# SewoongLab/PLeaS-Merging

Measured on NVIDIA B200. Metric: rn50_pair_merge_calib_samples_per_s, higher is better.
Workload: dtype f32

## Files before the change

### include/pleas_b200.h

```cpp
#ifndef PLEAS_B200_H
#define PLEAS_B200_H

#include <stdint.h>

#ifdef __cplusplus
extern "C" {
#endif

#define PLB_OK 0
#define PLB_EINVAL (-1)
#define PLB_ESIZE (-2)
#define PLB_EALIGN (-3)

#define PLB_MODE_INNER 0
#define PLB_MODE_NEG_CDIST 1
#define PLB_MODE_CORR 2

int plb_version(void);
const char *plb_last_error_string(void);


int64_t plb_plane_bytes(int64_t rows, int64_t K, int32_t *row_groups, int32_t *k_blocks);

int plb_pack_split(const float *x, int64_t outer, int64_t src_rows, int64_t inner,
                   const int64_t *row_index, int64_t rows,
                   float *hi, float *lo, int32_t row_groups, int32_t kb_offset,
                   double *row_sumsq, double *row_sum, void *stream);

int plb_pack_split_pair(const float *xa, const float *xb, int64_t outer, int64_t src_rows, int64_t inner,
                        float *hi_a, float *lo_a, float *hi_b, float *lo_b, int32_t row_groups,
                        int32_t kb_offset, double *sumsq_a, double *sumsq_b, void *stream);
int plb_pack_split_pair_sums(const float *xa, const float *xb, int64_t outer, int64_t src_rows, int64_t inner,
                             float *hi_a, float *lo_a, float *hi_b, float *lo_b, int32_t row_groups,
                             int32_t kb_offset, double *sumsq_a, double *sumsq_b, double *sum_a,
                             double *sum_b, void *stream);

int plb_pack_im2col(const float *x1, const float *x2, int64_t N, int64_t cin_src, int64_t H, int64_t W,
                    const int32_t *chan1, const int32_t *chan2, const float *scale1, const float *scale2,
                    int64_t cmerged, int32_t kh, int32_t kw, int32_t stride_h, int32_t stride_w,
                    int32_t pad_h, int32_t pad_w, int32_t dil_h, int32_t dil_w, int64_t Ho, int64_t Wo,
                    int32_t ones_row, float *hi, float *lo, int32_t row_groups, int32_t kb_offset,
                    void *stream);

int plb_gram_direct(const float *x, const float *y, int64_t outer, int64_t C, int64_t inner,
                    float *partial, int32_t splits, int32_t chain_kb, double *row_sumsq_x,
                    double *row_sumsq_y, void *stream);

int plb_gram_tma(const float *x, const float *y, int64_t outer, int64_t C, int64_t inner,
                 float *partial, int32_t splits, int32_t chain_kb, double *row_sumsq_x,
                 double *row_sumsq_y, double *row_sum_x, double *row_sum_y, void *stream);

int plb_debug_set_trace(unsigned long long *dev_buf);

int plb_gram_tma_geometry(int64_t C, int32_t *cta_group, int32_t *m_tiles, int32_t *n_tiles,
                          int32_t *ld_m, int32_t *ld_n);

typedef struct PlbGemmProblem {
  const float *a_hi, *a_lo;
  const float *b_hi, *b_lo;
  float *partial;
  int32_t a_row_groups, b_row_groups;
  int32_t k_blocks;
  int32_t m_tiles, n_tiles, splits;
  int32_t cta_begin;
  int32_t symmetric;
} PlbGemmProblem;

int plb_gemm_grouped(const PlbGemmProblem *problems_dev, int32_t n_problems, int32_t total_ctas,
                     int32_t bn, int32_t impl, void *stream);

int plb_cross_finalize(const float *partial, int32_t splits, int64_t ld_m, int64_t ld_n,
                       int64_t M, int64_t N, const double *qa, const double *qb, int32_t mode,
                       float *cost, double *cost64, int64_t ldc, int32_t accumulate, int32_t sym_bn,
                       void *stream);

typedef struct PlbFinalizeTap {
  const float *partial;
  const double *qa, *qb;
  const double *sa, *sb;
  int64_t ld_m, ld_n, K;
  int32_t splits;
  int32_t n_affine;
  const double *affine;
} PlbFinalizeTap;
typedef struct PlbFinalizeGroup {
  float *cost;
  int64_t ldc;
  int32_t n, tap_begin, tap_end, block_begin;
} PlbFinalizeGroup;
int plb_cross_finalize_grouped(const PlbFinalizeTap *taps_dev, const PlbFinalizeGroup *groups_dev,
                               int32_t n_groups, int32_t total_blocks, int32_t mode, int32_t accumulate,
                               void *stream);

int plb_cross_finalize_corr(const float *partial, int32_t splits, int64_t ld_m, int64_t ld_n,
                            int64_t M, int64_t N, const double *qa, const double *qb,
                            const double *sa, const double *sb, int64_t K, float *cost, int64_t ldc,
                            int32_t accumulate, void *stream);

int plb_lap_solve_batched(const float *const *cost, const int32_t *n, const int32_t *ld,
                          int64_t *const *col4row, double *objective, int32_t *status,
                          int32_t n_problems, int32_t max_n, int32_t maximize, void *stream);

int plb_lap_solve_batched_warm(const float *const *cost, const int32_t *n, const int32_t *ld,
                               int64_t *const *col4row, double *objective, int32_t *status,
                               int32_t n_problems, int32_t max_n, int32_t maximize,
                               const double *const *v_in, double v_scale, double *const *v_out, void *stream);


int plb_get_blocks(const float *cost, int64_t ldc, const int64_t *perm, int32_t n, float ratio,
                   int32_t identity, int64_t *q_merged, int64_t *p_merged, int64_t *q_sep,
                   int64_t *p_sep, int32_t *counts, void *stream);

int plb_block_merge(const float *w1, const float *w2, int64_t O, int64_t I, int64_t R,
                    const int64_t *bo1, const int64_t *bo2, const int64_t *bo1c, const int64_t *bo2c,
                    int64_t no, int64_t mo,
                    const int64_t *bi1, const int64_t *bi2, const int64_t *bi1c, const int64_t *bi2c,
                    int64_t ni, int64_t mi, int32_t in_axis_only, float *out, void *stream);

int plb_gather_axis(const float *in, float *out, int64_t outer, int64_t n, int64_t inner,
                    const int64_t *P, void *stream);

int plb_compose_perm(const int64_t *a, const int64_t *b, int64_t *out, int64_t n, void *stream);

int plb_wm_progress(const float *A, int64_t ld, const int64_t *P, int32_t n, int32_t *flag,
                    double *gain, void *stream);

int plb_conv_debug_set_trace(unsigned long long *dev_buf);
int64_t plb_conv_packed_floats(int64_t Cout, int64_t Cin, int32_t KH, int32_t KW);
int plb_conv_pack_weights(const float *w, int64_t Cout, int64_t Cin, int32_t KH, int32_t KW, float *packed,
                          void *stream);

int plb_conv2d_forward(const float *const *x, const float *const *packed_w, const float *const *bias,
                       float *const *out, int32_t nprob, int64_t NB, int64_t Cin, int64_t IH, int64_t IW,
                       int64_t Cout, int32_t KH, int32_t KW, int32_t stride, int32_t pad_h, int32_t pad_w,
                       void *stream);

int plb_conv2d_affine_forward(const float *const *x, const float *const *packed_w, const float *const *bias,
                              float *const *out, const float *const *scale_shift, float *const *out2,
                              int32_t relu, int32_t nprob, int64_t NB, int64_t Cin, int64_t IH, int64_t IW,
                              int64_t Cout, int32_t KH, int32_t KW, int32_t stride, int32_t pad_h, int32_t pad_w,
                              void *stream);

int plb_chol_solve(double *G, int64_t n, double *B, int64_t nrhs, double ridge, int32_t *info,
                   void *stream);

#ifdef __cplusplus
}
#endif
#endif
```

### pleas_merging_b200/_native.py

```python
import ctypes
import os

_HERE = os.path.dirname(os.path.abspath(__file__))
LIB_PATH = os.path.join(_HERE, "lib", "libpleas_b200.so")

c_i32, c_i64, c_f32, c_f64, c_ptr = ctypes.c_int32, ctypes.c_int64, ctypes.c_float, ctypes.c_double, ctypes.c_void_p


class GemmProblem(ctypes.Structure):
    _fields_ = [
        ("a_hi", c_ptr), ("a_lo", c_ptr), ("b_hi", c_ptr), ("b_lo", c_ptr), ("partial", c_ptr),
        ("a_row_groups", c_i32), ("b_row_groups", c_i32), ("k_blocks", c_i32),
        ("m_tiles", c_i32), ("n_tiles", c_i32), ("splits", c_i32), ("cta_begin", c_i32), ("symmetric", c_i32),
    ]


class FinalizeTap(ctypes.Structure):
    _fields_ = [("partial", c_ptr), ("qa", c_ptr), ("qb", c_ptr), ("sa", c_ptr), ("sb", c_ptr),
                ("ld_m", c_i64), ("ld_n", c_i64), ("K", c_i64), ("splits", c_i32), ("n_affine", c_i32),
                ("affine", c_ptr)]


class FinalizeGroup(ctypes.Structure):
    _fields_ = [("cost", c_ptr), ("ldc", c_i64), ("n", c_i32), ("tap_begin", c_i32), ("tap_end", c_i32),
                ("block_begin", c_i32)]


_SIGNATURES = {
    "plb_version": (ctypes.c_int, []),
    "plb_last_error_string": (ctypes.c_char_p, []),
    "plb_plane_bytes": (c_i64, [c_i64, c_i64, ctypes.POINTER(c_i32), ctypes.POINTER(c_i32)]),
    "plb_pack_split": (ctypes.c_int, [c_ptr, c_i64, c_i64, c_i64, c_ptr, c_i64, c_ptr, c_ptr, c_i32, c_i32,
                                      c_ptr, c_ptr, c_ptr]),
    "plb_pack_split_pair": (ctypes.c_int, [c_ptr, c_ptr, c_i64, c_i64, c_i64, c_ptr, c_ptr, c_ptr, c_ptr, c_i32, c_i32,
                                           c_ptr, c_ptr, c_ptr]),
    "plb_gram_direct": (ctypes.c_int, [c_ptr, c_ptr, c_i64, c_i64, c_i64, c_ptr, c_i32, c_i32, c_ptr, c_ptr, c_ptr]),
    "plb_gram_tma": (ctypes.c_int, [c_ptr, c_ptr, c_i64, c_i64, c_i64, c_ptr, c_i32, c_i32, c_ptr, c_ptr, c_ptr, c_ptr,
                                    c_ptr]),
    "plb_pack_split_pair_sums": (ctypes.c_int, [c_ptr, c_ptr, c_i64, c_i64, c_i64, c_ptr, c_ptr, c_ptr, c_ptr, c_i32,
                                                c_i32, c_ptr, c_ptr, c_ptr, c_ptr, c_ptr]),
    "plb_cross_finalize_grouped": (ctypes.c_int, [c_ptr, c_ptr, c_i32, c_i32, c_i32, c_i32, c_ptr]),
    "plb_cross_finalize_corr": (ctypes.c_int, [c_ptr, c_i32, c_i64, c_i64, c_i64, c_i64, c_ptr, c_ptr, c_ptr, c_ptr,
                                               c_i64, c_ptr, c_i64, c_i32, c_ptr]),
    "plb_gram_tma_geometry": (ctypes.c_int, [c_i64, ctypes.POINTER(c_i32), ctypes.POINTER(c_i32),
                                             ctypes.POINTER(c_i32), ctypes.POINTER(c_i32), ctypes.POINTER(c_i32)]),
    "plb_debug_set_trace": (ctypes.c_int, [c_ptr]),
    "plb_pack_im2col": (ctypes.c_int, [c_ptr, c_ptr, c_i64, c_i64, c_i64, c_i64, c_ptr, c_ptr, c_ptr, c_ptr, c_i64,
                                       c_i32, c_i32, c_i32, c_i32, c_i32, c_i32, c_i32, c_i32, c_i64, c_i64, c_i32,
                                       c_ptr, c_ptr, c_i32, c_i32, c_ptr]),
    "plb_gemm_grouped": (ctypes.c_int, [c_ptr, c_i32, c_i32, c_i32, c_i32, c_ptr]),
    "plb_cross_finalize": (ctypes.c_int, [c_ptr, c_i32, c_i64, c_i64, c_i64, c_i64, c_ptr, c_ptr, c_i32, c_ptr,
                                          c_ptr, c_i64, c_i32, c_i32, c_ptr]),
    "plb_lap_solve_batched": (ctypes.c_int, [c_ptr, c_ptr, c_ptr, c_ptr, c_ptr, c_ptr, c_i32, c_i32, c_i32, c_ptr]),
    "plb_lap_solve_batched_warm": (ctypes.c_int, [c_ptr, c_ptr, c_ptr, c_ptr, c_ptr, c_ptr, c_i32, c_i32, c_i32, c_ptr,
                                                  c_f64, c_ptr, c_ptr]),
    "plb_get_blocks": (ctypes.c_int, [c_ptr, c_i64, c_ptr, c_i32, c_f32, c_i32, c_ptr, c_ptr, c_ptr, c_ptr, c_ptr,
                                      c_ptr]),
    "plb_block_merge": (ctypes.c_int, [c_ptr, c_ptr, c_i64, c_i64, c_i64, c_ptr, c_ptr, c_ptr, c_ptr, c_i64, c_i64,
                                       c_ptr, c_ptr, c_ptr, c_ptr, c_i64, c_i64, c_i32, c_ptr, c_ptr]),
    "plb_gather_axis": (ctypes.c_int, [c_ptr, c_ptr, c_i64, c_i64, c_i64, c_ptr, c_ptr]),
    "plb_compose_perm": (ctypes.c_int, [c_ptr, c_ptr, c_ptr, c_i64, c_ptr]),
    "plb_wm_progress": (ctypes.c_int, [c_ptr, c_i64, c_ptr, c_i32, c_ptr, c_ptr, c_ptr]),
    "plb_chol_solve": (ctypes.c_int, [c_ptr, c_i64, c_ptr, c_i64, c_f64, c_ptr, c_ptr]),
    "plb_conv_debug_set_trace": (ctypes.c_int, [c_ptr]),
    "plb_conv_packed_floats": (c_i64, [c_i64, c_i64, c_i32, c_i32]),
    "plb_conv_pack_weights": (ctypes.c_int, [c_ptr, c_i64, c_i64, c_i32, c_i32, c_ptr, c_ptr]),
    "plb_conv2d_forward": (ctypes.c_int, [c_ptr, c_ptr, c_ptr, c_ptr, c_i32, c_i64, c_i64, c_i64, c_i64, c_i64,
                                          c_i32, c_i32, c_i32, c_i32, c_i32, c_ptr]),
    "plb_conv2d_affine_forward": (ctypes.c_int, [c_ptr, c_ptr, c_ptr, c_ptr, c_ptr, c_ptr, c_i32, c_i32, c_i64, c_i64,
                                                 c_i64, c_i64, c_i64, c_i32, c_i32, c_i32, c_i32, c_i32, c_ptr]),
}

EXPORTED_SYMBOLS = tuple(_SIGNATURES)
_lib = None


def lib():
    global _lib
    if _lib is None:
        if not os.path.exists(LIB_PATH):
            raise RuntimeError(
                f"pleas_merging_b200: CUDA library not found at {LIB_PATH}; build it with "
                "`python -m pleas_merging_b200.build` (or __graft_entry__.build()). There is no CPU fallback.")
        handle = ctypes.CDLL(LIB_PATH)
        for name, (res, args) in _SIGNATURES.items():
            fn = getattr(handle, name)
            fn.restype, fn.argtypes = res, args
        _lib = handle
    return _lib


import collections

LAUNCH_COUNTS = collections.Counter()


def check(rc, what):
    LAUNCH_COUNTS[what] += 1
    if rc != 0:
        msg = lib().plb_last_error_string().decode(errors="replace")
        raise RuntimeError(f"pleas_merging_b200: {what} failed with status {rc}: {msg}")


def call(name, device, *args):
    import torch

    fn = getattr(lib(), name)
    if device.index is None or device.index == torch.cuda.current_device():
        rc = fn(*args, torch.cuda.current_stream().cuda_stream)
    else:
        with torch.cuda.device(device):
            rc = fn(*args, torch.cuda.current_stream(device).cuda_stream)
    check(rc, name)


def stream_ptr(device=None):
    import torch

    return torch.cuda.current_stream(device).cuda_stream


_SM_COUNT = {}


def sm_count(device=None):
    import torch

    idx = torch.cuda.current_device() if device is None or getattr(device, "index", None) is None else device.index
    if idx not in _SM_COUNT:
        _SM_COUNT[idx] = torch.cuda.get_device_properties(idx).multi_processor_count
    return _SM_COUNT[idx]


def ptr(t):
    return None if t is None else t.data_ptr()
```

### pleas_merging_b200/csrc/conv.cu

```cuda
#include "tma.cuh"

namespace plb {

constexpr int kConvStages = 4;
constexpr int kConvThreads = 576;
constexpr int kConvMaxFlatK = 512;

struct ConvParams {
  const float *x[2];
  const float *bias[2];
  float *out[2];
  const float2 *post[2];
  float *out2[2];
  int post_relu;
  int nprob;
  int NB, Cin, IH, IW, Cout, OH, OW, KH, KW, stride, pad_h, pad_w;
  int P, OHW, IHW;
  int m_tiles, n_tiles, total_items;
  int taps;
  int nbox;
  int flat;
  int flat_groups;
  int flat_lg;
  int chain_boxes;
  unsigned long long *trace;
  int debug;
};

__device__ __forceinline__ void tmem_st16(uint32_t taddr, const uint32_t (&v)[16]) {
  asm volatile(
      "tcgen05.st.sync.aligned.32x32b.x16.b32 [%0], "
      "{%1, %2, %3, %4, %5, %6, %7, %8, %9, %10, %11, %12, %13, %14, %15, %16};" ::"r"(taddr),
      "r"(v[0]), "r"(v[1]), "r"(v[2]), "r"(v[3]), "r"(v[4]), "r"(v[5]), "r"(v[6]), "r"(v[7]), "r"(v[8]), "r"(v[9]),
      "r"(v[10]), "r"(v[11]), "r"(v[12]), "r"(v[13]), "r"(v[14]), "r"(v[15])
      : "memory");
}
__device__ __forceinline__ void tmem_st_wait() { asm volatile("tcgen05.wait::st.sync.aligned;" ::: "memory"); }
__device__ __forceinline__ void tmem_ld16(uint32_t taddr, uint32_t (&v)[16]) {
  asm volatile(
      "tcgen05.ld.sync.aligned.32x32b.x16.b32 "
      "{%0, %1, %2, %3, %4, %5, %6, %7, %8, %9, %10, %11, %12, %13, %14, %15}, [%16];"
      : "=r"(v[0]), "=r"(v[1]), "=r"(v[2]), "=r"(v[3]), "=r"(v[4]), "=r"(v[5]), "=r"(v[6]), "=r"(v[7]),
        "=r"(v[8]), "=r"(v[9]), "=r"(v[10]), "=r"(v[11]), "=r"(v[12]), "=r"(v[13]), "=r"(v[14]), "=r"(v[15])
      : "r"(taddr));
}
__device__ __forceinline__ void umma_tf32_ts(uint32_t tmem_d, uint32_t tmem_a, uint64_t bdesc, uint32_t idesc,
                                             uint32_t accumulate) {
  asm volatile(
      "{\n\t.reg .pred p;\n\t"
      "setp.ne.b32 p, %4, 0;\n\t"
      "tcgen05.mma.cta_group::1.kind::tf32 [%0], [%1], %2, %3, p;\n\t}" ::"r"(tmem_d),
      "r"(tmem_a), "l"(bdesc), "r"(idesc), "r"(accumulate)
      : "memory");
}
__device__ __forceinline__ void tma_load_4d(void *smem_dst, const CUtensorMap *map, int c0, int c1, int c2, int c3,
                                            uint64_t *bar) {
  asm volatile(
      "cp.async.bulk.tensor.4d.shared::cluster.global.tile.mbarrier::complete_tx::bytes [%0], [%1, {%2, %3, %4, %5}], "
      "[%6];" ::"r"(smem_u32(smem_dst)),
      "l"(map), "r"(c0), "r"(c1), "r"(c2), "r"(c3), "r"(smem_u32(bar))
      : "memory");
}

template <int TN>
struct ConvCfg {
  static constexpr int kBBytes = kConvStages * 2 * TN * 128;
  static constexpr int kARing = TN == 128 ? 5 : 8;
  static constexpr int kSmemBytes = kBBytes + kARing * 16384 + 1024;
};

__device__ __forceinline__ void cp_async4(uint32_t smem_dst, const float *src, uint32_t ignore) {
  asm volatile(
      "{\n\t.reg .pred p;\n\t"
      "setp.ne.b32 p, %2, 0;\n\t"
      "cp.async.ca.shared.global [%0], [%1], 4, p;\n\t}" ::"r"(smem_dst),
      "l"(src), "r"(ignore)
      : "memory");
}
__device__ __forceinline__ void cp_async_commit() { asm volatile("cp.async.commit_group;" ::: "memory"); }
template <int N>
__device__ __forceinline__ void cp_async_wait() {
  asm volatile("cp.async.wait_group %0;" ::"n"(N) : "memory");
}

__device__ __forceinline__ uint32_t opaque_smem_u32(const void *p) {
  uint32_t a;
  asm volatile("{\n\t.reg .u64 t;\n\tcvta.to.shared.u64 t, %1;\n\tcvt.u32.u64 %0, t;\n\t}" : "=r"(a) : "l"(p));
  return a;
}
__device__ __forceinline__ void a32_expect_tx(uint32_t bar, uint32_t bytes) {
  asm volatile("mbarrier.arrive.expect_tx.shared::cta.b64 _, [%0], %1;" ::"r"(bar), "r"(bytes) : "memory");
}
__device__ __forceinline__ void a32_arrive(uint32_t bar) {
  asm volatile("mbarrier.arrive.shared::cta.b64 _, [%0];" ::"r"(bar) : "memory");
}
__device__ __forceinline__ bool a32_try_wait(uint32_t bar, uint32_t parity) {
  uint32_t ok;
  asm volatile(
      "{\n\t.reg .pred P;\n\t"
      "mbarrier.try_wait.parity.shared::cta.b64 P, [%1], %2;\n\t"
      "selp.b32 %0, 1, 0, P;\n\t}"
      : "=r"(ok)
      : "r"(bar), "r"(parity)
      : "memory");
  return ok != 0;
}
__device__ __forceinline__ bool a32_test_wait(uint32_t bar, uint32_t parity) {
  uint32_t ok;
  asm volatile(
      "{\n\t.reg .pred P;\n\t"
      "mbarrier.test_wait.parity.shared::cta.b64 P, [%1], %2;\n\t"
      "selp.b32 %0, 1, 0, P;\n\t}"
      : "=r"(ok)
      : "r"(bar), "r"(parity)
      : "memory");
  return ok != 0;
}
__device__ __forceinline__ void a32_wait_wd(uint32_t bar, uint32_t parity) {
  if (a32_try_wait(bar, parity)) return;
  const long long t0 = clock64();
  while (!a32_try_wait(bar, parity))
    if (clock64() - t0 > kWatchdogClocks) __trap();
}
__device__ __forceinline__ void a32_commit(uint32_t bar) {
  asm volatile("tcgen05.commit.cta_group::1.mbarrier::arrive::one.shared::cluster.b64 [%0];" ::"r"(bar) : "memory");
}
__device__ __forceinline__ void a32_tma_load_4d(uint32_t smem_dst, const CUtensorMap *map, int c0, int c1, int c2,
                                                int c3, uint32_t bar) {
  asm volatile(
      "cp.async.bulk.tensor.4d.shared::cluster.global.tile.mbarrier::complete_tx::bytes [%0], [%1, {%2, %3, %4, %5}], "
      "[%6];" ::"r"(smem_dst),
      "l"(map), "r"(c0), "r"(c1), "r"(c2), "r"(c3), "r"(bar)
      : "memory");
}

template <int LG>
__device__ __forceinline__ void flat_rows(const int2 *rows, const float *origin, const float *safe, uint32_t dst,
                                          bool pvalid, int ih0, int iw0, int IH, int IW, int KW) {
  constexpr int TAPS = 1 << LG, ROWS = 16 >> LG;
#pragma unroll
  for (int r = 0; r < ROWS; ++r) {
    const int2 e = rows[r];
    const bool rowok = pvalid && e.y >= 0 && (unsigned)(ih0 + e.y) < (unsigned)IH;
    const float *base = rowok ? origin + e.x : safe;
#pragma unroll
    for (int t = 0; t < TAPS; ++t) {
      const bool ok = rowok && t < KW && (unsigned)(iw0 + t) < (unsigned)IW;
      cp_async4(dst + (r * TAPS + t) * 512, base + (ok ? t : 0), ok ? 0u : 1u);
    }
  }
}

template <int COLS, bool BIAS, bool POST>
__device__ __forceinline__ void store_tile(const float (&acc)[COLS], float *o, float *o2, int ohw, const float *bias,
                                           const float2 *ss, bool relu, int) {
#pragma unroll
  for (int c = 0; c < COLS; ++c) {
    const float v = acc[c];
    o[(int64_t)c * ohw] = v;
    if (POST) {
      const float2 a = __ldg(ss + c);
      const float w = fmaf(v, a.x, a.y);
      o2[(int64_t)c * ohw] = relu ? fmaxf(w, 0.f) : w;
    }
  }
}
template <int COLS>
__device__ __noinline__ void store_tile_ragged(const float (&acc)[COLS], float *o, float *o2, int ohw, const float *bias,
                                               const float2 *ss, bool relu, int nc) {
#pragma unroll 4
  for (int c = 0; c < COLS; ++c) {
    if (c >= nc) break;
    const float v = acc[c] + (bias ? __ldg(bias + c) : 0.f);
    o[(int64_t)c * ohw] = v;
    if (o2 != nullptr) {
      const float2 a = __ldg(ss + c);
      const float w = fmaf(v, a.x, a.y);
      o2[(int64_t)c * ohw] = relu ? fmaxf(w, 0.f) : w;
    }
  }
}

struct ConvItem {
  int prob, mt, nt;
};
__device__ __forceinline__ ConvItem conv_item(const ConvParams &p, int item) {
  ConvItem it;
  it.nt = item % p.n_tiles;
  const int rest = item / p.n_tiles;
  it.prob = rest % p.nprob;
  it.mt = rest / p.nprob;
  return it;
}

template <int TN, int CH, bool DBG>
__global__ void __launch_bounds__(kConvThreads, 1) conv3xtf32_kernel(const __grid_constant__ CUtensorMap tmw0,
                                                                      const __grid_constant__ CUtensorMap tmw1,
                                                                      ConvParams p) {
  constexpr int kPlaneBytes = TN * 128;
  constexpr int kStageBytes = 2 * kPlaneBytes;
  constexpr uint32_t kACol0 = 2 * TN;
  constexpr int kARing = ConvCfg<TN>::kARing;
  extern __shared__ uint8_t smem_raw[];
  __shared__ uint64_t bars[2 * kConvStages + 4];
  __shared__ uint32_t tmem_base_s;
  __shared__ int2 ktab[kConvMaxFlatK];

  uint8_t *smem = (uint8_t *)(((uintptr_t)smem_raw + 1023) & ~(uintptr_t)1023);
  const int warp = threadIdx.x >> 5, lane = threadIdx.x & 31;
  const int cta = (int)blockIdx.x, nctas = (int)gridDim.x;
  const uint32_t bars_a = opaque_smem_u32(bars), smem_a = opaque_smem_u32(smem);
  const uint32_t bar_full = bars_a, bar_empty = bars_a + 8 * kConvStages, bar_acc_full = bars_a + 16 * kConvStages,
                 bar_acc_empty = bar_acc_full + 16;

  if (warp == 0 && lane == 0) {
    for (int s = 0; s < kConvStages; ++s) {
      mbar_init(&bars[s], 1 + 8);
      mbar_init(&bars[kConvStages + s], 1);
    }
    for (int b = 0; b < 2; ++b) {
      mbar_init(&bars[2 * kConvStages + b], 1);
      mbar_init(&bars[2 * kConvStages + 2 + b], 8);
    }
    fence_mbar_init();
  } else if (warp == 1) {
    tmem_alloc(&tmem_base_s, 512);
    tmem_relinquish();
  }
  if (p.flat) {
    const int rows = (p.nbox * 32) >> p.flat_lg;
    for (int g = (int)threadIdx.x; g < rows; g += kConvThreads) {
      int2 e;
      if (g < p.flat_groups) {
        const int ci = g / p.KH, kh = g - ci * p.KH;
        e.x = ci * p.IHW + kh * p.IW;
        e.y = kh;
      } else {
        e.x = 0;
        e.y = -1;
      }
      ktab[g] = e;
    }
  }
  tc_fence_before();
  __syncthreads();
  tc_fence_after();
  const uint32_t tmem_base = tmem_base_s;

  if (warp == 0) {
    uint32_t i = 0;
    for (int item = cta; item < p.total_items; item += nctas) {
      const ConvItem it = conv_item(p, item);
      const CUtensorMap *map = it.prob ? &tmw1 : &tmw0;
      const int n0 = it.nt * TN;
      int cb = 0, tap = 0;
      for (int b = 0; b < p.nbox; ++b, ++i) {
        const uint32_t s = i & (kConvStages - 1), ph = (i / kConvStages) & 1u;
        a32_wait_wd(bar_empty + 8 * s, ph ^ 1u);
        if (DBG && p.trace && cta == 0 && lane == 0 && i < 512) p.trace[i * 16 + 0] = clock64();
        if (elect_one()) {
          const uint32_t st = smem_a + s * kStageBytes;
          a32_expect_tx(bar_full + 8 * s, kStageBytes);
          a32_tma_load_4d(st, map, cb * 32, n0, tap, 0, bar_full + 8 * s);
          a32_tma_load_4d(st + kPlaneBytes, map, cb * 32, n0, tap, 1, bar_full + 8 * s);
        }
        __syncwarp();
        if (++tap == p.taps) {
          tap = 0;
          ++cb;
        }
      }
    }
  } else if (warp == 1) {
    constexpr uint32_t idesc = umma_idesc_tf32(128, TN);
    const uint32_t smem_base = smem_a;
    uint32_t i = 0, chain = 0;
    uint32_t ready = 0;
    bool acc_ok = false;
    for (int item = cta; item < p.total_items; item += nctas) {
      for (int b0 = 0; b0 < p.nbox; b0 += CH, ++chain) {
        const uint32_t buf = chain & 1u;
        const int nb = min(CH, p.nbox - b0);
        const bool trm = DBG && p.trace && cta == 0 && lane == 0 && i < 512;
        if (trm) p.trace[i * 16 + 8] = clock64();
        if (!acc_ok) a32_wait_wd(bar_acc_empty + 8 * buf, ((chain >> 1) & 1u) ^ 1u);
        const uint32_t d_tmem = tmem_base + buf * TN;
#pragma unroll
        for (int q = 0; q < CH; ++q)
          if (q < nb && !((ready >> q) & 1u)) a32_wait_wd(bar_full + 8 * ((i + q) & (kConvStages - 1)), ((i + q) / kConvStages) & 1u);
        if (trm) p.trace[i * 16 + 4] = clock64();
        tc_fence_after();
        if (elect_one()) {
#pragma unroll
          for (int q = 0; q < CH; ++q) {
            if (q >= nb) break;
            const uint32_t s = (i + q) & (kConvStages - 1);
            const uint32_t bst = smem_base + s * kStageBytes, a_hi0 = tmem_base + kACol0 + s * 64;
#pragma unroll
            for (int j = 0; j < 4; ++j) {
              umma_tf32_ts(d_tmem, a_hi0 + 32 + 8 * j, umma_desc_sw<128>(bst + 32 * j), idesc, (q > 0 || j > 0) ? 1u : 0u);
              if (!(DBG && p.debug & 2))
                umma_tf32_ts(d_tmem, a_hi0 + 8 * j, umma_desc_sw<128>(bst + kPlaneBytes + 32 * j), idesc, 1u);
            }
          }
        }
        __syncwarp();
        uint32_t nready = 0;
#pragma unroll
        for (int q = 0; q < CH; ++q) {
          const uint32_t in = i + nb + q;
          if (a32_test_wait(bar_full + 8 * (in & (kConvStages - 1)), (in / kConvStages) & 1u)) nready |= 1u << q;
        }
        const bool next_acc = a32_test_wait(bar_acc_empty + 8 * ((chain + 1) & 1u), (((chain + 1) >> 1) & 1u) ^ 1u);
        if (elect_one()) {
#pragma unroll
          for (int q = 0; q < CH; ++q) {
            if (q >= nb) break;
            const uint32_t s = (i + q) & (kConvStages - 1);
            const uint32_t bst = smem_base + s * kStageBytes, a_hi0 = tmem_base + kACol0 + s * 64;
            if (!(DBG && p.debug & 2)) {
#pragma unroll
              for (int j = 0; j < 4; ++j) umma_tf32_ts(d_tmem, a_hi0 + 8 * j, umma_desc_sw<128>(bst + 32 * j), idesc, 1u);
            }
            a32_commit(bar_empty + 8 * s);
          }
          a32_commit(bar_acc_full + 8 * buf);
        }
        ready = __reduce_and_sync(0xffffffffu, nready);
        acc_ok = __all_sync(0xffffffffu, next_acc);
        if (trm) p.trace[i * 16 + 6] = clock64();
        i += nb;
      }
    }
  } else if (warp < 10) {
    const int hsel = (warp - 2) >> 2;
    const int row = (warp & 3) * 32 + lane;
    const uint32_t a_base = tmem_base + ((uint32_t)((warp & 3) * 32) << 16) + kACol0 + 16 * hsel;
    const uint32_t ring = smem_a + ConvCfg<TN>::kBBytes + (uint32_t)(hsel * 16) * 512u + (uint32_t)row * 4u;
    const int my_items = cta < p.total_items ? (p.total_items - cta + nctas - 1) / nctas : 0;
    const int total = my_items * p.nbox;
    const int kh_n = p.flat ? 1 : p.KH, kw_n = p.flat ? 1 : p.KW, cb_n = p.nbox / (kh_n * kw_n);
    int itx = 0, cb = 0, kh = 0, kw = 0, ih0 = 0, iw0 = 0;
    bool pvalid = false;
    const float *xn = nullptr;
    auto locate = [&]() {
      const ConvItem it = conv_item(p, cta + itx * nctas);
      const int pos = it.mt * 128 + row;
      pvalid = pos < p.P;
      const int n = pvalid ? pos / p.OHW : 0, r = pos - n * p.OHW, oh = r / p.OW, ow = r - oh * p.OW;
      ih0 = oh * p.stride - p.pad_h;
      iw0 = ow * p.stride - p.pad_w;
      xn = p.x[it.prob] + (int64_t)n * p.Cin * p.IHW;
    };
    if (total > 0) locate();

    auto issue = [&](int slot) {
      const uint32_t dst = ring + (uint32_t)slot * 16384u;
      if (!p.flat) {
        const int ih = ih0 + kh, iw = iw0 + kw;
        const bool ok = pvalid && (unsigned)ih < (unsigned)p.IH && (unsigned)iw < (unsigned)p.IW;
        const float *src = ok ? xn + (int64_t)(cb * 32 + hsel * 16) * p.IHW + ih * p.IW + iw : xn;
        const uint32_t cs = ok ? (uint32_t)p.IHW : 0u, ign = ok ? 0u : 1u;
#pragma unroll
        for (int c = 0; c < 16; ++c) cp_async4(dst + c * 512, src + (uint32_t)c * cs, ign);
      } else {
        const int row0 = (cb * 32 + hsel * 16) >> p.flat_lg;
        const float *origin = xn + ih0 * p.IW + iw0;
        switch (p.flat_lg) {
          case 0: flat_rows<0>(ktab + row0, origin, xn, dst, pvalid, ih0, iw0, p.IH, p.IW, p.KW); break;
          case 1: flat_rows<1>(ktab + row0, origin, xn, dst, pvalid, ih0, iw0, p.IH, p.IW, p.KW); break;
          case 2: flat_rows<2>(ktab + row0, origin, xn, dst, pvalid, ih0, iw0, p.IH, p.IW, p.KW); break;
          case 3: flat_rows<3>(ktab + row0, origin, xn, dst, pvalid, ih0, iw0, p.IH, p.IW, p.KW); break;
          default: flat_rows<4>(ktab + row0, origin, xn, dst, pvalid, ih0, iw0, p.IH, p.IW, p.KW); break;
        }
      }
      if (++kw == kw_n) {
        kw = 0;
        if (++kh == kh_n) {
          kh = 0;
          if (++cb == cb_n) {
            cb = 0;
            ++itx;
            if (itx < my_items) locate();
          }
        }
      }
    };

    int slot_in = 0;
#pragma unroll 1
    for (int j = 0; j < kARing - 1; ++j) {
      if (j < total && !(DBG && p.debug & 1)) issue(slot_in);
      cp_async_commit();
      if (++slot_in == kARing) slot_in = 0;
    }
    int slot_out = 0;
#pragma unroll 1
    for (int i = 0; i < total; ++i) {
      if (i + kARing - 1 < total && !(DBG && p.debug & 1)) issue(slot_in);
      cp_async_commit();
      if (++slot_in == kARing) slot_in = 0;
      cp_async_wait<kARing - 1>();
      uint32_t v[16];
#pragma unroll
      for (int c = 0; c < 16; ++c)
        asm volatile("ld.shared.b32 %0, [%1];" : "=r"(v[c]) : "r"(ring + (uint32_t)slot_out * 16384u + c * 512u) : "memory");
      if (++slot_out == kARing) slot_out = 0;
      const uint32_t s = (uint32_t)i & (kConvStages - 1), ph = ((uint32_t)i / kConvStages) & 1u;
      const bool tr = DBG && p.trace && cta == 0 && warp == 2 && lane == 0 && i < 512;
      a32_wait_wd(bar_empty + 8 * s, ph ^ 1u);
      tc_fence_after();
      uint32_t hi[16];
#pragma unroll
      for (int c = 0; c < 16; ++c) hi[c] = (v[c] + 0x1000u) & 0xffffe000u;
      tmem_st16(a_base + s * 64, hi);
#pragma unroll
      for (int c = 0; c < 16; ++c)
        hi[c] = __float_as_uint(__uint_as_float(v[c]) - __uint_as_float(hi[c])) + 0x1000u;
      tmem_st16(a_base + s * 64 + 32, hi);
      tmem_st_wait();
      if (tr) p.trace[i * 16 + 3] = clock64();
      tc_fence_before();
      __syncwarp();
      if (lane == 0) a32_arrive(bar_full + 8 * s);
    }
  } else {
    constexpr int COLS = TN / 2;
    const int q = warp & 3;
    const int half = (warp - 10) >> 2;
    uint32_t chain = 0;
    for (int item = cta; item < p.total_items; item += nctas) {
      const ConvItem it = conv_item(p, item);
      unsigned long long acc2[COLS / 2];
#pragma unroll
      for (int c = 0; c < COLS / 2; ++c) acc2[c] = 0ull;
      for (int b0 = 0; b0 < p.nbox; b0 += CH, ++chain) {
        const uint32_t buf = chain & 1u;
        a32_wait_wd(bar_acc_full + 8 * buf, (chain >> 1) & 1u);
        const bool tr = DBG && p.trace && cta == 0 && warp == 10 && lane == 0 && chain < 512;
        if (tr) p.trace[chain * 16 + 5] = clock64();
        tc_fence_after();
        const uint32_t t0 = tmem_base + ((uint32_t)(q * 32) << 16) + buf * TN + half * COLS;
#pragma unroll
        for (int c = 0; c < COLS / 16; ++c) {
          uint32_t v[16];
          tmem_ld16(t0 + c * 16, v);
          tmem_ld_wait();
#pragma unroll
          for (int e = 0; e < 8; ++e) {
            unsigned long long pr;
            asm("mov.b64 %0, {%1, %2};" : "=l"(pr) : "r"(v[2 * e]), "r"(v[2 * e + 1]));
            asm("add.rn.f32x2 %0, %0, %1;" : "+l"(acc2[c * 8 + e]) : "l"(pr));
          }
        }
        tc_fence_before();
        __syncwarp();
        if (lane == 0) a32_arrive(bar_acc_empty + 8 * buf);
        if (tr) p.trace[chain * 16 + 7] = clock64();
      }
      float acc[COLS];
#pragma unroll
      for (int c = 0; c < COLS / 2; ++c) {
        uint32_t lo, hi;
        asm("mov.b64 {%0, %1}, %2;" : "=r"(lo), "=r"(hi) : "l"(acc2[c]));
        acc[2 * c] = __uint_as_float(lo);
        acc[2 * c + 1] = __uint_as_float(hi);
      }
      const int pos = it.mt * 128 + q * 32 + lane;
      if (pos < p.P && !(DBG && p.debug & 4)) {
        const int n = pos / p.OHW, r = pos - n * p.OHW;
        const int co0 = it.nt * TN + half * COLS;
        float *o = p.out[it.prob] + ((int64_t)n * p.Cout + co0) * p.OHW + r;
        const float *bias = p.bias[it.prob];
        const int ohw = p.OHW;
        const int nc = min(COLS, p.Cout - co0);
        float *o2 = p.out2[it.prob] ? p.out2[it.prob] + ((int64_t)n * p.Cout + co0) * p.OHW + r : nullptr;
        const float2 *ss = p.post[it.prob] ? p.post[it.prob] + co0 : nullptr;
        const bool relu = p.post_relu != 0;
        if (nc == COLS && bias == nullptr && o2 == nullptr) {
          store_tile<COLS, false, false>(acc, o, o2, ohw, bias, ss, relu, nc);
        } else if (nc == COLS && bias == nullptr) {
          store_tile<COLS, false, true>(acc, o, o2, ohw, bias, ss, relu, nc);
        } else {
          store_tile_ragged<COLS>(acc, o, o2, ohw, bias ? bias + co0 : nullptr, ss, relu, nc);
        }
      }
    }
  }

  tc_fence_before();
  __syncthreads();
  if (warp == 1) tmem_dealloc(tmem_base, 512);
}

__global__ void conv_pack_weights_kernel(const float *__restrict__ w, float *__restrict__ packed, int Cout, int Cin,
                                         int KH, int KW, int taps, int Kc, int flat, int flat_lg) {
  const int64_t plane = (int64_t)taps * Cout * Kc;
  for (int64_t idx = (int64_t)blockIdx.x * blockDim.x + threadIdx.x; idx < plane; idx += (int64_t)gridDim.x * blockDim.x) {
    const int k = (int)(idx % Kc);
    const int co = (int)((idx / Kc) % Cout);
    const int t = (int)(idx / ((int64_t)Kc * Cout));
    float v = 0.f;
    if (!flat) {
      v = w[((int64_t)co * Cin + k) * (KH * KW) + t];
    } else {
      const int g = k >> flat_lg, kw = k & ((1 << flat_lg) - 1);
      if (g < Cin * KH && kw < KW) v = w[((int64_t)co * Cin * KH + g) * KW + kw];
    }
    const float hi = to_tf32(v);
    packed[idx] = hi;
    packed[plane + idx] = to_tf32(v - hi);
  }
}

static unsigned long long *g_conv_trace = nullptr;

struct ConvGeometry {
  int flat, taps, Kc, flat_lg;
};
static ConvGeometry conv_geometry(int64_t Cin, int KH, int KW) {
  ConvGeometry g;
  g.flat = (Cin % 32) != 0;
  g.taps = g.flat ? 1 : KH * KW;
  g.flat_lg = 0;
  while ((1 << g.flat_lg) < KW) ++g.flat_lg;
  g.Kc = g.flat ? (int)(ceil_div((Cin * KH) << g.flat_lg, 32) * 32) : (int)Cin;
  return g;
}

static int make_weight_map(CUtensorMap *m, const float *packed, int64_t Cout, const ConvGeometry &g, int tn) {
  EncodeTiledFn enc = encode_tiled();
  PLB_REQUIRE(enc != nullptr, PLB_EINVAL, "plb_conv2d_forward: cuTensorMapEncodeTiled is not available from this driver");
  cuuint64_t gdim[4] = {(cuuint64_t)g.Kc, (cuuint64_t)Cout, (cuuint64_t)g.taps, 2};
  cuuint64_t gstride[3] = {(cuuint64_t)g.Kc * 4, (cuuint64_t)g.Kc * Cout * 4, (cuuint64_t)g.Kc * Cout * g.taps * 4};
  cuuint32_t box[4] = {32, (cuuint32_t)tn, 1, 1};
  cuuint32_t estr[4] = {1, 1, 1, 1};
  CUresult r = enc(m, CU_TENSOR_MAP_DATA_TYPE_FLOAT32, 4, (void *)packed, gdim, gstride, box, estr,
                   CU_TENSOR_MAP_INTERLEAVE_NONE, CU_TENSOR_MAP_SWIZZLE_128B, CU_TENSOR_MAP_L2_PROMOTION_L2_256B,
                   CU_TENSOR_MAP_FLOAT_OOB_FILL_NONE);
  PLB_REQUIRE(r == CUDA_SUCCESS, PLB_EINVAL, "plb_conv2d_forward: cuTensorMapEncodeTiled failed with CUresult %d", (int)r);
  return PLB_OK;
}

template <int TN, int CH, bool DBG>
static int launch_conv(const CUtensorMap &m0, const CUtensorMap &m1, const ConvParams &p, cudaStream_t stream) {
  constexpr int smem_bytes = ConvCfg<TN>::kSmemBytes;
  if (int rc = ensure_dynamic_smem((const void *)conv3xtf32_kernel<TN, CH, DBG>, smem_bytes, "conv3xtf32_kernel"))
    return rc;
  const int grid = min(p.total_items, device_sm_count());
  conv3xtf32_kernel<TN, CH, DBG><<<grid, kConvThreads, smem_bytes, stream>>>(m0, m1, p);
  return launch_status("conv3xtf32_kernel");
}

}

extern "C" int plb_conv_debug_set_trace(unsigned long long *dev_buf) {
  plb::g_conv_trace = dev_buf;
  return PLB_OK;
}

extern "C" int64_t plb_conv_packed_floats(int64_t Cout, int64_t Cin, int32_t KH, int32_t KW) {
  if (Cout <= 0 || Cin <= 0 || KH <= 0 || KW <= 0) return 0;
  const plb::ConvGeometry g = plb::conv_geometry(Cin, KH, KW);
  return 2ll * g.taps * Cout * g.Kc;
}

extern "C" int plb_conv_pack_weights(const float *w, int64_t Cout, int64_t Cin, int32_t KH, int32_t KW, float *packed,
                                     void *stream) {
  using namespace plb;
  PLB_REQUIRE(w && packed, PLB_EINVAL, "plb_conv_pack_weights: null pointer");
  PLB_REQUIRE(Cout > 0 && Cin > 0 && KH > 0 && KW > 0, PLB_EINVAL, "plb_conv_pack_weights: empty weight");
  const ConvGeometry g = conv_geometry(Cin, KH, KW);
  PLB_REQUIRE(!g.flat || KW <= 16, PLB_ESIZE, "plb_conv_pack_weights: Cin %% 32 != 0 needs KW <= 16");
  PLB_REQUIRE(!g.flat || g.Kc <= kConvMaxFlatK, PLB_ESIZE,
              "plb_conv_pack_weights: Cin %% 32 != 0 needs Cin*KH*pow2(KW) <= %d", kConvMaxFlatK);
  const int64_t plane = (int64_t)g.taps * Cout * g.Kc;
  PLB_REQUIRE(plane < (1ll << 31), PLB_ESIZE, "plb_conv_pack_weights: weight too large");
  const int64_t want = ceil_div(plane, 256);
  const int blocks = (int)(want < 148 * 8 ? want : 148 * 8);
  conv_pack_weights_kernel<<<blocks, 256, 0, (cudaStream_t)stream>>>(w, packed, (int)Cout, (int)Cin, KH, KW, g.taps,
                                                                     g.Kc, g.flat, g.flat_lg);
  return launch_status("conv_pack_weights_kernel");
}

extern "C" int plb_conv2d_forward(const float *const *x, const float *const *packed_w, const float *const *bias,
                                  float *const *out, int32_t nprob, int64_t NB, int64_t Cin, int64_t IH, int64_t IW,
                                  int64_t Cout, int32_t KH, int32_t KW, int32_t stride, int32_t pad_h, int32_t pad_w,
                                  void *stream) {
  return plb_conv2d_affine_forward(x, packed_w, bias, out, nullptr, nullptr, 0, nprob, NB, Cin, IH, IW, Cout, KH, KW,
                                   stride, pad_h, pad_w, stream);
}

extern "C" int plb_conv2d_affine_forward(const float *const *x, const float *const *packed_w,
                                         const float *const *bias, float *const *out,
                                         const float *const *scale_shift, float *const *out2, int32_t relu,
                                         int32_t nprob, int64_t NB, int64_t Cin, int64_t IH, int64_t IW, int64_t Cout,
                                         int32_t KH, int32_t KW, int32_t stride, int32_t pad_h, int32_t pad_w,
                                         void *stream) {
  using namespace plb;
  PLB_REQUIRE(x && packed_w && out, PLB_EINVAL, "plb_conv2d_forward: null pointer table");
  PLB_REQUIRE(nprob == 1 || nprob == 2, PLB_EINVAL, "plb_conv2d_forward: one or two problems per launch");
  PLB_REQUIRE(NB > 0 && Cin > 0 && IH > 0 && IW > 0 && Cout > 0 && KH > 0 && KW > 0 && stride > 0 && pad_h >= 0 &&
                  pad_w >= 0,
              PLB_EINVAL, "plb_conv2d_forward: bad geometry");
  const int64_t OH = (IH + 2 * pad_h - KH) / stride + 1, OW = (IW + 2 * pad_w - KW) / stride + 1;
  PLB_REQUIRE(OH > 0 && OW > 0, PLB_EINVAL, "plb_conv2d_forward: empty output");
  PLB_REQUIRE(NB * OH * OW < (1ll << 31) - 128 && NB * Cin * IH * IW < (1ll << 40) && Cin * IH * IW < (1ll << 31) &&
                  KH < 256 && KW < 256,
              PLB_ESIZE, "plb_conv2d_forward: extent too large");
  const ConvGeometry g = conv_geometry(Cin, KH, KW);
  PLB_REQUIRE(!g.flat || KW <= 16, PLB_ESIZE, "plb_conv2d_forward: Cin %% 32 != 0 needs KW <= 16");
  PLB_REQUIRE(!g.flat || g.Kc <= kConvMaxFlatK, PLB_ESIZE,
              "plb_conv2d_forward: Cin %% 32 != 0 needs Cin*KH*pow2(KW) <= %d", kConvMaxFlatK);
  ConvParams p = {};
  for (int i = 0; i < nprob; ++i) {
    PLB_REQUIRE(x[i] && packed_w[i] && out[i], PLB_EINVAL, "plb_conv2d_forward: null pointer");
    PLB_REQUIRE(((uintptr_t)packed_w[i] & 15) == 0, PLB_EALIGN, "plb_conv2d_forward: packed weights must be 16-byte aligned");
    p.x[i] = x[i];
    p.out[i] = out[i];
    p.bias[i] = bias ? bias[i] : nullptr;
    PLB_REQUIRE((scale_shift == nullptr) == (out2 == nullptr) &&
                    (out2 == nullptr || ((scale_shift[i] != nullptr) && (out2[i] != nullptr))),
                PLB_EINVAL, "plb_conv2d_affine_forward: scale_shift and out2 go together");
    PLB_REQUIRE(scale_shift == nullptr || ((uintptr_t)scale_shift[i] & 7) == 0, PLB_EALIGN,
                "plb_conv2d_affine_forward: scale_shift must be 8-byte aligned");
    p.post[i] = scale_shift ? reinterpret_cast<const float2 *>(scale_shift[i]) : nullptr;
    p.out2[i] = out2 ? out2[i] : nullptr;
  }
  p.nprob = nprob;
  p.post_relu = relu;
  p.NB = (int)NB, p.Cin = (int)Cin, p.IH = (int)IH, p.IW = (int)IW, p.Cout = (int)Cout, p.OH = (int)OH, p.OW = (int)OW;
  p.KH = KH, p.KW = KW, p.stride = stride, p.pad_h = pad_h, p.pad_w = pad_w;
  p.P = (int)(NB * OH * OW), p.OHW = (int)(OH * OW), p.IHW = (int)(IH * IW);
  p.flat = g.flat, p.taps = g.taps, p.flat_groups = (int)(Cin * KH), p.flat_lg = g.flat_lg;
  p.nbox = g.taps * (g.Kc / 32);
  static int debug = -1;
  if (debug < 0) {
    const char *d = getenv("PLB_CONV_DEBUG");
    debug = d ? atoi(d) : 0;
  }
  p.debug = debug;
  p.trace = g_conv_trace;
  static int chain = 0;
  if (chain == 0) {
    const char *c = getenv("PLB_CONV_CHAIN");
    chain = (c && atoi(c) > 0 && atoi(c) <= kConvStages / 2) ? atoi(c) : 2;
  }
  p.chain_boxes = chain;
  const int tn = Cout <= 64 ? 64 : 128;
  p.m_tiles = (int)ceil_div(p.P, 128);
  p.n_tiles = (int)ceil_div(Cout, tn);
  const int64_t items = (int64_t)p.m_tiles * p.n_tiles * nprob;
  PLB_REQUIRE(items * p.nbox < (1ll << 31), PLB_ESIZE, "plb_conv2d_forward: too many work items");
  p.total_items = (int)items;
  CUtensorMap m0, m1;
  if (int rc = make_weight_map(&m0, packed_w[0], Cout, g, tn)) return rc;
  if (int rc = make_weight_map(&m1, packed_w[nprob - 1], Cout, g, tn)) return rc;
  cudaStream_t s = (cudaStream_t)stream;
  const bool dbg = p.debug != 0 || p.trace != nullptr;
  if (dbg || chain != 2) {
    if (chain == 1) return tn == 64 ? launch_conv<64, 1, true>(m0, m1, p, s) : launch_conv<128, 1, true>(m0, m1, p, s);
    return tn == 64 ? launch_conv<64, 2, true>(m0, m1, p, s) : launch_conv<128, 2, true>(m0, m1, p, s);
  }
  return tn == 64 ? launch_conv<64, 2, false>(m0, m1, p, s) : launch_conv<128, 2, false>(m0, m1, p, s);
}
```

Before: 2702.

## Add split-K with in-kernel fixup to conv kernel for underfilled waves

```diff
diff --git a/include/pleas_b200.h b/include/pleas_b200.h
--- a/include/pleas_b200.h
+++ b/include/pleas_b200.h
@@ -130,6 +130,9 @@
 int plb_conv_pack_weights(const float *w, int64_t Cout, int64_t Cin, int32_t KH, int32_t KW, float *packed,
                           void *stream);
 
+int32_t plb_conv_split_count(int64_t NB, int64_t Cin, int64_t IH, int64_t IW, int64_t Cout, int32_t KH, int32_t KW,
+                             int32_t stride, int32_t pad_h, int32_t pad_w, int32_t sms);
+
 int plb_conv2d_forward(const float *const *x, const float *const *packed_w, const float *const *bias,
                        float *const *out, int32_t nprob, int64_t NB, int64_t Cin, int64_t IH, int64_t IW,
                        int64_t Cout, int32_t KH, int32_t KW, int32_t stride, int32_t pad_h, int32_t pad_w,
diff --git a/pleas_merging_b200/_native.py b/pleas_merging_b200/_native.py
--- a/pleas_merging_b200/_native.py
+++ b/pleas_merging_b200/_native.py
@@ -65,6 +65,7 @@
     "plb_conv_debug_set_trace": (ctypes.c_int, [c_ptr]),
     "plb_conv_packed_floats": (c_i64, [c_i64, c_i64, c_i32, c_i32]),
     "plb_conv_pack_weights": (ctypes.c_int, [c_ptr, c_i64, c_i64, c_i32, c_i32, c_ptr, c_ptr]),
+    "plb_conv_split_count": (c_i32, [c_i64, c_i64, c_i64, c_i64, c_i64, c_i32, c_i32, c_i32, c_i32, c_i32, c_i32]),
     "plb_conv2d_forward": (ctypes.c_int, [c_ptr, c_ptr, c_ptr, c_ptr, c_i32, c_i64, c_i64, c_i64, c_i64, c_i64,
                                           c_i32, c_i32, c_i32, c_i32, c_i32, c_ptr]),
     "plb_conv2d_affine_forward": (ctypes.c_int, [c_ptr, c_ptr, c_ptr, c_ptr, c_ptr, c_ptr, c_i32, c_i32, c_i64, c_i64,
diff --git a/pleas_merging_b200/csrc/conv.cu b/pleas_merging_b200/csrc/conv.cu
--- a/pleas_merging_b200/csrc/conv.cu
+++ b/pleas_merging_b200/csrc/conv.cu
@@ -1,3 +1,7 @@
+#include <algorithm>
+#include <map>
+#include <mutex>
+
 #include "tma.cuh"
 
 namespace plb {
@@ -5,6 +9,8 @@
 constexpr int kConvStages = 4;
 constexpr int kConvThreads = 576;
 constexpr int kConvMaxFlatK = 512;
+constexpr int kConvMaxSplits = 4;
+constexpr int kConvMinSplitChains = 12;
 
 struct ConvParams {
   const float *x[2];
@@ -23,6 +29,9 @@
   int flat_groups;
   int flat_lg;
   int chain_boxes;
+  int splits;
+  float *partial;
+  unsigned *tile_count;
   unsigned long long *trace;
   int debug;
 };
@@ -182,18 +191,67 @@
 }
 
 struct ConvItem {
-  int prob, mt, nt;
+  int prob, mt, nt, split;
 };
+template <bool SPLIT>
 __device__ __forceinline__ ConvItem conv_item(const ConvParams &p, int item) {
   ConvItem it;
-  it.nt = item % p.n_tiles;
-  const int rest = item / p.n_tiles;
+  it.split = SPLIT ? item % p.splits : 0;
+  const int tile = SPLIT ? item / p.splits : item;
+  it.nt = tile % p.n_tiles;
+  const int rest = tile / p.n_tiles;
   it.prob = rest % p.nprob;
   it.mt = rest / p.nprob;
   return it;
 }
 
-template <int TN, int CH, bool DBG>
+template <int CH, bool SPLIT>
+__device__ __forceinline__ int2 split_boxes(const ConvParams &p, int split) {
+  if (!SPLIT) return make_int2(0, p.nbox);
+  const int chains = (p.nbox + CH - 1) / CH;
+  return make_int2(split * chains / p.splits * CH, min((split + 1) * chains / p.splits * CH, p.nbox));
+}
+
+__device__ __forceinline__ void epilogue_bar_sync() { asm volatile("bar.sync 1, 256;" ::: "memory"); }
+
+template <int TN>
+__device__ __forceinline__ bool split_fixup(const ConvParams &p, int item, int split, int row, int half,
+                                            float (&acc)[TN / 2], int *last_s) {
+  constexpr int Q = TN / 8;
+  const int tile = item / p.splits;
+  float4 *w = reinterpret_cast<float4 *>(p.partial) + ((int64_t)tile * p.splits * (TN / 4) + half * Q) * 128 + row;
+#pragma unroll
+  for (int j = 0; j < Q; ++j)
+    __stcg(w + ((int64_t)split * (TN / 4) + j) * 128, make_float4(acc[4 * j], acc[4 * j + 1], acc[4 * j + 2], acc[4 * j + 3]));
+  epilogue_bar_sync();
+  if (threadIdx.x == 10 * 32) {
+    __threadfence();
+    const unsigned old = atomicAdd(p.tile_count + tile, 1u);
+    const int last = old == (unsigned)p.splits - 1;
+    if (last) {
+      p.tile_count[tile] = 0;
+      __threadfence();
+    }
+    *last_s = last;
+  }
+  epilogue_bar_sync();
+  if (!*last_s) return false;
+#pragma unroll
+  for (int j = 0; j < Q; ++j) {
+    float4 t = __ldcg(w + j * 128);
+#pragma unroll
+    for (int s = 1; s < kConvMaxSplits; ++s) {
+      if (s < p.splits) {
+        const float4 v = __ldcg(w + ((int64_t)s * (TN / 4) + j) * 128);
+        t.x += v.x, t.y += v.y, t.z += v.z, t.w += v.w;
+      }
+    }
+    acc[4 * j] = t.x, acc[4 * j + 1] = t.y, acc[4 * j + 2] = t.z, acc[4 * j + 3] = t.w;
+  }
+  return true;
+}
+
+template <int TN, int CH, bool DBG, bool SPLIT>
 __global__ void __launch_bounds__(kConvThreads, 1) conv3xtf32_kernel(const __grid_constant__ CUtensorMap tmw0,
                                                                       const __grid_constant__ CUtensorMap tmw1,
                                                                       ConvParams p) {
@@ -204,6 +262,7 @@
   extern __shared__ uint8_t smem_raw[];
   __shared__ uint64_t bars[2 * kConvStages + 4];
   __shared__ uint32_t tmem_base_s;
+  __shared__ int fix_last;
   __shared__ int2 ktab[kConvMaxFlatK];
 
   uint8_t *smem = (uint8_t *)(((uintptr_t)smem_raw + 1023) & ~(uintptr_t)1023);
@@ -250,11 +309,12 @@
   if (warp == 0) {
     uint32_t i = 0;
     for (int item = cta; item < p.total_items; item += nctas) {
-      const ConvItem it = conv_item(p, item);
+      const ConvItem it = conv_item<SPLIT>(p, item);
       const CUtensorMap *map = it.prob ? &tmw1 : &tmw0;
       const int n0 = it.nt * TN;
-      int cb = 0, tap = 0;
-      for (int b = 0; b < p.nbox; ++b, ++i) {
+      const int2 br = split_boxes<CH, SPLIT>(p, it.split);
+      int cb = br.x / p.taps, tap = br.x - cb * p.taps;
+      for (int b = br.x; b < br.y; ++b, ++i) {
         const uint32_t s = i & (kConvStages - 1), ph = (i / kConvStages) & 1u;
         a32_wait_wd(bar_empty + 8 * s, ph ^ 1u);
         if (DBG && p.trace && cta == 0 && lane == 0 && i < 512) p.trace[i * 16 + 0] = clock64();
@@ -278,9 +338,10 @@
     uint32_t ready = 0;
     bool acc_ok = false;
     for (int item = cta; item < p.total_items; item += nctas) {
-      for (int b0 = 0; b0 < p.nbox; b0 += CH, ++chain) {
+      const int2 br = split_boxes<CH, SPLIT>(p, SPLIT ? item % p.splits : 0);
+      for (int b0 = br.x; b0 < br.y; b0 += CH, ++chain) {
         const uint32_t buf = chain & 1u;
-        const int nb = min(CH, p.nbox - b0);
+        const int nb = min(CH, br.y - b0);
         const bool trm = DBG && p.trace && cta == 0 && lane == 0 && i < 512;
         if (trm) p.trace[i * 16 + 8] = clock64();
         if (!acc_ok) a32_wait_wd(bar_acc_empty + 8 * buf, ((chain >> 1) & 1u) ^ 1u);
@@ -338,13 +399,23 @@
     const uint32_t a_base = tmem_base + ((uint32_t)((warp & 3) * 32) << 16) + kACol0 + 16 * hsel;
     const uint32_t ring = smem_a + ConvCfg<TN>::kBBytes + (uint32_t)(hsel * 16) * 512u + (uint32_t)row * 4u;
     const int my_items = cta < p.total_items ? (p.total_items - cta + nctas - 1) / nctas : 0;
-    const int total = my_items * p.nbox;
+    int total = SPLIT ? 0 : my_items * p.nbox;
+    for (int item = cta; SPLIT && item < p.total_items; item += nctas) {
+      const int2 br = split_boxes<CH, SPLIT>(p, SPLIT ? item % p.splits : 0);
+      total += br.y - br.x;
+    }
     const int kh_n = p.flat ? 1 : p.KH, kw_n = p.flat ? 1 : p.KW, cb_n = p.nbox / (kh_n * kw_n);
-    int itx = 0, cb = 0, kh = 0, kw = 0, ih0 = 0, iw0 = 0;
+    int itx = 0, cb = 0, kh = 0, kw = 0, left = 0, ih0 = 0, iw0 = 0;
     bool pvalid = false;
     const float *xn = nullptr;
     auto locate = [&]() {
-      const ConvItem it = conv_item(p, cta + itx * nctas);
+      const ConvItem it = conv_item<SPLIT>(p, cta + itx * nctas);
+      const int2 br = split_boxes<CH, SPLIT>(p, it.split);
+      cb = br.x / (kh_n * kw_n);
+      const int tap = br.x - cb * (kh_n * kw_n);
+      kh = tap / kw_n;
+      kw = tap - kh * kw_n;
+      left = br.y - br.x;
       const int pos = it.mt * 128 + row;
       pvalid = pos < p.P;
       const int n = pvalid ? pos / p.OHW : 0, r = pos - n * p.OHW, oh = r / p.OW, ow = r - oh * p.OW;
@@ -378,13 +449,10 @@
         kw = 0;
         if (++kh == kh_n) {
           kh = 0;
-          if (++cb == cb_n) {
-            cb = 0;
-            ++itx;
-            if (itx < my_items) locate();
-          }
+          if (++cb == cb_n && !SPLIT && ++itx < my_items) locate();
         }
       }
+      if (SPLIT && --left == 0 && ++itx < my_items) locate();
     };
 
     int slot_in = 0;
@@ -430,11 +498,12 @@
     const int half = (warp - 10) >> 2;
     uint32_t chain = 0;
     for (int item = cta; item < p.total_items; item += nctas) {
-      const ConvItem it = conv_item(p, item);
+      const ConvItem it = conv_item<SPLIT>(p, item);
       unsigned long long acc2[COLS / 2];
 #pragma unroll
       for (int c = 0; c < COLS / 2; ++c) acc2[c] = 0ull;
-      for (int b0 = 0; b0 < p.nbox; b0 += CH, ++chain) {
+      const int2 br = split_boxes<CH, SPLIT>(p, it.split);
+      for (int b0 = br.x; b0 < br.y; b0 += CH, ++chain) {
         const uint32_t buf = chain & 1u;
         a32_wait_wd(bar_acc_full + 8 * buf, (chain >> 1) & 1u);
         const bool tr = DBG && p.trace && cta == 0 && warp == 10 && lane == 0 && chain < 512;
@@ -466,6 +535,7 @@
         acc[2 * c] = __uint_as_float(lo);
         acc[2 * c + 1] = __uint_as_float(hi);
       }
+      if (SPLIT && p.splits > 1 && !split_fixup<TN>(p, item, it.split, q * 32 + lane, half, acc, &fix_last)) continue;
       const int pos = it.mt * 128 + q * 32 + lane;
       if (pos < p.P && !(DBG && p.debug & 4)) {
         const int n = pos / p.OHW, r = pos - n * p.OHW;
@@ -528,6 +598,64 @@
   return g;
 }
 
+static int conv_chain_boxes() {
+  static int chain = 0;
+  if (chain == 0) {
+    const char *c = getenv("PLB_CONV_CHAIN");
+    chain = (c && atoi(c) > 0 && atoi(c) <= kConvStages / 2) ? atoi(c) : 2;
+  }
+  return chain;
+}
+
+static int conv_splits(int64_t tiles, int nbox, int chain, int sms) {
+  const int64_t items = 2 * tiles, chains = ceil_div(nbox, chain);
+  int64_t waves = ceil_div(items, sms);
+  if (items * 10 >= waves * sms * 9) return 1;
+  int best = 1;
+  for (int s = 2; s <= kConvMaxSplits && chains >= (int64_t)s * kConvMinSplitChains; ++s) {
+    const int64_t w = ceil_div(items * s, sms);
+    if (w * best < waves * s) best = s, waves = w;
+  }
+  return best;
+}
+
+struct ConvWorkspace {
+  unsigned *count = nullptr;
+  float *partial = nullptr;
+  int64_t count_cap = 0, partial_cap = 0;
+};
+static int conv_workspace(int64_t counters, int64_t floats, cudaStream_t stream, ConvWorkspace *out) {
+  static std::mutex mu;
+  static std::map<int, ConvWorkspace> ws;
+  int dev = 0;
+  cudaError_t e = cudaGetDevice(&dev);
+  PLB_REQUIRE(e == cudaSuccess, (int)e, "plb_conv2d_forward: cudaGetDevice: %s", cudaGetErrorString(e));
+  std::lock_guard<std::mutex> lock(mu);
+  ConvWorkspace &w = ws[dev];
+  if (w.count_cap < counters || w.partial_cap < floats) {
+    cudaStreamCaptureStatus cs = cudaStreamCaptureStatusNone;
+    cudaStreamIsCapturing(stream, &cs);
+    PLB_REQUIRE(cs == cudaStreamCaptureStatusNone, PLB_EINVAL,
+                "plb_conv2d_forward: the split-K workspace (%lld floats) must be allocated by an eager call of this "
+                "shape before graph capture", (long long)floats);
+    ConvWorkspace n;
+    n.count_cap = std::max(counters, w.count_cap);
+    n.partial_cap = std::max(floats, w.partial_cap);
+    const int64_t count_bytes = ceil_div(n.count_cap * 4, 256) * 256;
+    void *base = nullptr;
+    e = cudaMalloc(&base, count_bytes + n.partial_cap * 4);
+    PLB_REQUIRE(e == cudaSuccess, (int)e, "plb_conv2d_forward: split-K workspace of %lld bytes: %s",
+                (long long)(count_bytes + n.partial_cap * 4), cudaGetErrorString(e));
+    e = cudaMemsetAsync(base, 0, count_bytes, stream);
+    PLB_REQUIRE(e == cudaSuccess, (int)e, "plb_conv2d_forward: cudaMemsetAsync: %s", cudaGetErrorString(e));
+    n.count = (unsigned *)base;
+    n.partial = (float *)((char *)base + count_bytes);
+    w = n;
+  }
+  *out = w;
+  return PLB_OK;
+}
+
 static int make_weight_map(CUtensorMap *m, const float *packed, int64_t Cout, const ConvGeometry &g, int tn) {
   EncodeTiledFn enc = encode_tiled();
   PLB_REQUIRE(enc != nullptr, PLB_EINVAL, "plb_conv2d_forward: cuTensorMapEncodeTiled is not available from this driver");
@@ -542,13 +670,13 @@
   return PLB_OK;
 }
 
-template <int TN, int CH, bool DBG>
+template <int TN, int CH, bool DBG, bool SPLIT>
 static int launch_conv(const CUtensorMap &m0, const CUtensorMap &m1, const ConvParams &p, cudaStream_t stream) {
   constexpr int smem_bytes = ConvCfg<TN>::kSmemBytes;
-  if (int rc = ensure_dynamic_smem((const void *)conv3xtf32_kernel<TN, CH, DBG>, smem_bytes, "conv3xtf32_kernel"))
+  if (int rc = ensure_dynamic_smem((const void *)conv3xtf32_kernel<TN, CH, DBG, SPLIT>, smem_bytes, "conv3xtf32_kernel"))
     return rc;
   const int grid = min(p.total_items, device_sm_count());
-  conv3xtf32_kernel<TN, CH, DBG><<<grid, kConvThreads, smem_bytes, stream>>>(m0, m1, p);
+  conv3xtf32_kernel<TN, CH, DBG, SPLIT><<<grid, kConvThreads, smem_bytes, stream>>>(m0, m1, p);
   return launch_status("conv3xtf32_kernel");
 }
 
@@ -581,6 +709,17 @@
   conv_pack_weights_kernel<<<blocks, 256, 0, (cudaStream_t)stream>>>(w, packed, (int)Cout, (int)Cin, KH, KW, g.taps,
                                                                      g.Kc, g.flat, g.flat_lg);
   return launch_status("conv_pack_weights_kernel");
+}
+
+extern "C" int32_t plb_conv_split_count(int64_t NB, int64_t Cin, int64_t IH, int64_t IW, int64_t Cout, int32_t KH,
+                                        int32_t KW, int32_t stride, int32_t pad_h, int32_t pad_w, int32_t sms) {
+  using namespace plb;
+  if (NB <= 0 || Cin <= 0 || Cout <= 0 || KH <= 0 || KW <= 0 || stride <= 0 || sms <= 0) return 0;
+  const int64_t OH = (IH + 2 * pad_h - KH) / stride + 1, OW = (IW + 2 * pad_w - KW) / stride + 1;
+  if (OH <= 0 || OW <= 0) return 0;
+  const ConvGeometry g = conv_geometry(Cin, KH, KW);
+  const int64_t tiles = ceil_div(NB * OH * OW, 128) * ceil_div(Cout, Cout <= 64 ? 64 : 128);
+  return conv_splits(tiles, g.taps * (g.Kc / 32), conv_chain_boxes(), sms);
 }
 
 extern "C" int plb_conv2d_forward(const float *const *x, const float *const *packed_w, const float *const *bias,
@@ -641,26 +780,32 @@
   }
   p.debug = debug;
   p.trace = g_conv_trace;
-  static int chain = 0;
-  if (chain == 0) {
-    const char *c = getenv("PLB_CONV_CHAIN");
-    chain = (c && atoi(c) > 0 && atoi(c) <= kConvStages / 2) ? atoi(c) : 2;
-  }
+  const int chain = conv_chain_boxes();
   p.chain_boxes = chain;
   const int tn = Cout <= 64 ? 64 : 128;
   p.m_tiles = (int)ceil_div(p.P, 128);
   p.n_tiles = (int)ceil_div(Cout, tn);
-  const int64_t items = (int64_t)p.m_tiles * p.n_tiles * nprob;
-  PLB_REQUIRE(items * p.nbox < (1ll << 31), PLB_ESIZE, "plb_conv2d_forward: too many work items");
-  p.total_items = (int)items;
+  const int64_t tiles = (int64_t)p.m_tiles * p.n_tiles * nprob;
+  PLB_REQUIRE(tiles * p.nbox < (1ll << 31), PLB_ESIZE, "plb_conv2d_forward: too many work items");
+  p.splits = conv_splits((int64_t)p.m_tiles * p.n_tiles, p.nbox, chain, device_sm_count());
+  p.total_items = (int)(tiles * p.splits);
+  cudaStream_t s = (cudaStream_t)stream;
+  if (p.splits > 1) {
+    ConvWorkspace ws;
+    if (int rc = conv_workspace(tiles, tiles * p.splits * 128 * tn, s, &ws)) return rc;
+    p.partial = ws.partial;
+    p.tile_count = ws.count;
+  }
   CUtensorMap m0, m1;
   if (int rc = make_weight_map(&m0, packed_w[0], Cout, g, tn)) return rc;
   if (int rc = make_weight_map(&m1, packed_w[nprob - 1], Cout, g, tn)) return rc;
-  cudaStream_t s = (cudaStream_t)stream;
   const bool dbg = p.debug != 0 || p.trace != nullptr;
   if (dbg || chain != 2) {
-    if (chain == 1) return tn == 64 ? launch_conv<64, 1, true>(m0, m1, p, s) : launch_conv<128, 1, true>(m0, m1, p, s);
-    return tn == 64 ? launch_conv<64, 2, true>(m0, m1, p, s) : launch_conv<128, 2, true>(m0, m1, p, s);
-  }
-  return tn == 64 ? launch_conv<64, 2, false>(m0, m1, p, s) : launch_conv<128, 2, false>(m0, m1, p, s);
-}
+    if (chain == 1)
+      return tn == 64 ? launch_conv<64, 1, true, true>(m0, m1, p, s) : launch_conv<128, 1, true, true>(m0, m1, p, s);
+    return tn == 64 ? launch_conv<64, 2, true, true>(m0, m1, p, s) : launch_conv<128, 2, true, true>(m0, m1, p, s);
+  }
+  if (p.splits > 1)
+    return tn == 64 ? launch_conv<64, 2, false, true>(m0, m1, p, s) : launch_conv<128, 2, false, true>(m0, m1, p, s);
+  return tn == 64 ? launch_conv<64, 2, false, false>(m0, m1, p, s) : launch_conv<128, 2, false, false>(m0, m1, p, s);
+}
```

After: 2683 (median of 6 runs). About the same (-0.7%).
